# ivan-digital/qwen3-asr-swift

Hardware: AMD Instinct MI355X
Metric: audio-seconds/sec (RTF^-1) Qwen3-ASR-0.6B, 30 s@16 kHz, b=32 per GPU (higher is better)
Workload: dtype bf16; 1 GPU; Qwen3-ASR-0.6B geometry (bf16), 32 clips x 30 s per GPU (BASELINE metric's b=32; x8 GPUs = configs[2]), timed region = pcm in host memory -> mel + encoder + prompt pass + 128 forced greedy tokens -> token ids in host memory, tokens gathered over RCCL; clips_per_gpu=32, weights=bf16

## Files before the change

### qwen3-asr-swift_amd/csrc/dec_kernels.h

```cpp
#pragma once
#include "common.h"
#include "gemm.h"
#include "dec_rope.h"
#include <vector>

namespace qasr {

struct QuantRaw {
    const uint32_t* wq = nullptr;
    const void* scales = nullptr;
    const void* biases = nullptr;
    int sb_f32 = 0;
    int N = 0, K = 0, bits = 0;
};

void rmsnorm_rows_launch(const bf16_t* x, const bf16_t* w, bf16_t* y, int rows, int H, float eps, hipStream_t s);

void embed_splice_launch(const int* ids, const int* audio_src, const bf16_t* embed, const bf16_t* audio, bf16_t* x,
                         int n_pos, int H, hipStream_t s);

void gather_rows_launch(const bf16_t* src, const int* row_idx, bf16_t* dst, int n, int H, hipStream_t s);

struct KVLayout {
    bf16_t* k;
    bf16_t* v;
    int max_ctx, kv_heads, hd;
    bf16_t* vf = nullptr;
    __host__ __device__ long off(int slot, int kvh, int pos) const {
        return (((long)slot * kv_heads + kvh) * max_ctx + pos) * hd;
    }
};

void qk_norm_rope_launch(const bf16_t* qkv, const int* slot, const int* pos, int n_pos, int heads, int kv_heads,
                         int hd, const bf16_t* qn_w, const bf16_t* kn_w, float eps, const float* rope_cos,
                         const float* rope_sin, bf16_t* qr, KVLayout cache, bf16_t* vt, int vt_stride,
                         const int* cu, const int* slot_of_clip, int n_clips, int max_len, hipStream_t s, bool v_only = false);
bool qk_norm_rope_fusable(int heads, int kv_heads, int hd);

void prefill_attention_launch(const bf16_t* qr, KVLayout cache, const bf16_t* vt, int vt_stride, const int* cu,
                              const int* slot_of_clip, int n_clips, int max_len, int heads, bf16_t* out,
                              hipStream_t s, unsigned long long* dbg = nullptr);

enum DecEpi { DEC_EPI_BF16 = 0, DEC_EPI_RESID = 1, DEC_EPI_SWIGLU = 2, DEC_EPI_LOGITS = 3 };

struct DecGemvArgs {
    const bf16_t* W;
    const bf16_t* Wp;
    const bf16_t* X;
    int B, N, K;
    bf16_t* out;
    float* logits;
    float* part_val;
    int* part_idx;
};
int decode_gemv_launch(DecEpi epi, const DecGemvArgs& a, hipStream_t s);
int decode_gemv_blocks(DecEpi epi, int N);
void argmax_rows_launch(const bf16_t* x, long ld, int rows, int n, int* out, hipStream_t s);

void decode_gemv_set_debug(unsigned long long* dbg);
int decode_gemv_fused_launch(DecEpi epi, const DecGemvArgs& a, const bf16_t* norm_w, float eps, bf16_t* norm_scratch,
                             hipStream_t s);
void decode_gemv_note_route(int tuned);
int decode_gemv_last_route();

// ... 15 lines not shown
    int* ctx_len;
    int* n_active;
    int* err;
    int max_new;
    int max_tokens;
    int eos;
    int ignore_eos;
    int vocab;
    unsigned* clear = nullptr;
    int clear_words = 0;
};
struct RopeRows {
    const float* cos_table; const float* sin_table;
    float* cos_rows; float* sin_rows;
    int half;
};
void greedy_finalize_launch(const float* part_val, const int* part_idx, int n_parts, GreedyState st, int B,
                            int advance_ctx, const bf16_t* embed, bf16_t* x, int H, RopeRows rr, hipStream_t s,
                            const QuantRaw* qembed = nullptr);

void refresh_rope_rows_launch(const int* ctx_len, RopeRows rr, int B, hipStream_t s);
void rope_tables_host(float theta, int half, int n_pos, std::vector<float>& c, std::vector<float>& sn);

struct EpiQkHeads {
    bf16_t* qkv; long ldo;
    bf16_t* qr;
    KVLayout cache;
    const int* slot; const int* pos;
    const bf16_t* qn_w; const bf16_t* kn_w;
    float eps;
    const float* rope_cos; const float* rope_sin;
    int heads, kv_heads;
    __device__ __forceinline__ bool head_tile(int n0) const { return n0 < (heads + kv_heads) * 128; }
    __device__ __forceinline__ void operator()(int m, int n, float4 v) const {
        *reinterpret_cast<uint2*>(qkv + (long)m * ldo + n) = pack_bf16x4(v);
    }
    __device__ __forceinline__ void rows(int m0, int n0, int M, const unsigned short* T, int tid) const {
        constexpr int HD = 128, HALF = 64;
        const int h = n0 / HD, j = tid & 7;
        const bf16_t* nw = h < heads ? qn_w : kn_w;
        const uint4 w1 = *reinterpret_cast<const uint4*>(nw + 8 * j), w2 = *reinterpret_cast<const uint4*>(nw + HALF + 8 * j);
        const bf16_t* w1e = reinterpret_cast<const bf16_t*>(&w1);
        const bf16_t* w2e = reinterpret_cast<const bf16_t*>(&w2);
#pragma unroll
        for (int pass = 0; pass < 4; ++pass) {
            const int row = pass * 32 + (tid >> 3);
            const bool live = m0 + row < M;
            const int m = live ? m0 + row : M - 1;
            const int sw = (row >> 2) & 7;
            const uint4 a = *reinterpret_cast<const uint4*>(T + row * 128 + ((j ^ sw) << 3));
            const uint4 b = *reinterpret_cast<const uint4*>(T + row * 128 + (((8 + j) ^ sw) << 3));
            const bf16_t* ae = reinterpret_cast<const bf16_t*>(&a);
            const bf16_t* be = reinterpret_cast<const bf16_t*>(&b);
            const int sl = slot[m], ps = pos[m];
            float x1[8], x2[8], ss = 0.0f;
#pragma unroll
            for (int e = 0; e < 8; ++e) {
                x1[e] = bf16_to_f32(ae[e]);
                x2[e] = bf16_to_f32(be[e]);
                ss += x1[e] * x1[e] + x2[e] * x2[e];
            }
#pragma unroll
            for (int ofs = 1; ofs < 8; ofs <<= 1) ss += __shfl_xor(ss, ofs, 64);
            const float inv = rsqrtf(ss / (float)HD + eps);
            const float4* cp = reinterpret_cast<const float4*>(rope_cos + (long)ps * HALF + 8 * j);
            const float4* sp = reinterpret_cast<const float4*>(rope_sin + (long)ps * HALF + 8 * j);
            const float4 c0 = cp[0], c1 = cp[1], s0 = sp[0], s1 = sp[1];
            const float cs[8] = {c0.x, c0.y, c0.z, c0.w, c1.x, c1.y, c1.z, c1.w};
            const float sn[8] = {s0.x, s0.y, s0.z, s0.w, s1.x, s1.y, s1.z, s1.w};
            uint4 o1, o2;
            bf16_t* o1e = reinterpret_cast<bf16_t*>(&o1);
            bf16_t* o2e = reinterpret_cast<bf16_t*>(&o2);
#pragma unroll
            for (int e = 0; e < 8; ++e) {
                float r1, r2;
                norm_rope_pair(x1[e], x2[e], bf16_to_f32(w1e[e]), bf16_to_f32(w2e[e]), inv, cs[e], sn[e], r1, r2);
                o1e[e] = f32_to_bf16(r1);
                o2e[e] = f32_to_bf16(r2);
            }
            if (live) {
                bf16_t* dst = h < heads ? qr + ((long)m * heads + h) * HD : cache.k + cache.off(sl, h - heads, ps);
                *reinterpret_cast<uint4*>(dst + 8 * j) = o1;
                *reinterpret_cast<uint4*>(dst + HALF + 8 * j) = o2;
            }
        }
    }
};

struct EpiResidBf16 {
    bf16_t* x; long ldx;
    struct Pre { uint2 r; };
    __device__ __forceinline__ Pre prefetch(int m, int n) const { return {*reinterpret_cast<const uint2*>(x + (long)m * ldx + n)}; }
    __device__ __forceinline__ void apply(int m, int n, float4 v, const Pre& p) const {
        float4 r = unpack_bf16x4(p.r);
        r.x += bf16_round(v.x); r.y += bf16_round(v.y); r.z += bf16_round(v.z); r.w += bf16_round(v.w);
        *reinterpret_cast<uint2*>(x + (long)m * ldx + n) = pack_bf16x4(r);
    }
    __device__ __forceinline__ void operator()(int m, int n, float4 v) const { apply(m, n, v, prefetch(m, n)); }
};

__device__ __forceinline__ float swiglu_bf16(float g_acc, float u_acc) { return gemm_swiglu(g_acc, u_acc); }

}
```

### qwen3-asr-swift_amd/csrc/dec_prefill.hip

```cpp
#include "dec_kernels.h"
#include "dec_rope.h"
#include <cstdlib>
#include <cstdio>

namespace qasr {

constexpr int RMS_MAXV = 4;

__global__ __launch_bounds__(256) void rmsnorm_rows_kernel(const bf16_t* __restrict__ x, const bf16_t* __restrict__ w,
                                                           bf16_t* __restrict__ y, int rows, int H, float eps) {
    const int row = blockIdx.x * 4 + (threadIdx.x >> 6), lane = threadIdx.x & 63;
    if (row >= rows) return;
    const int nch = H / 8;
    const uint4* xr = reinterpret_cast<const uint4*>(x + (long)row * H);
    uint4 v[RMS_MAXV];
    float ss = 0.0f;
#pragma unroll
    for (int i = 0; i < RMS_MAXV; ++i) {
        int c = lane + 64 * i;
        v[i] = c < nch ? xr[c] : make_uint4(0, 0, 0, 0);
        const bf16_t* e = reinterpret_cast<const bf16_t*>(&v[i]);
#pragma unroll
        for (int j = 0; j < 8; ++j) { float f = bf16_to_f32(e[j]); ss = fmaf(f, f, ss); }
    }
// ... 221 lines not shown
        long waves = (long)n_pos * (nh / 2);
        hipLaunchKernelGGL(qk_norm_rope_kernel<128>, dim3(cdiv(waves, 4)), dim3(256), 0, s, qkv, slot, pos, n_pos, heads,
                           kv_heads, qn_w, kn_w, eps, rope_cos, rope_sin, qr, cache);
        hipLaunchKernelGGL(v_transpose_kernel<128>, tgrid, dim3(256), 0, s, cache, qkv, nh, heads + kv_heads, cu, slot_of_clip, vt_out, vt_stride);
    } else if (hd == 32 && nh % 8 == 0) {
        long waves = (long)n_pos * (nh / 8);
        hipLaunchKernelGGL(qk_norm_rope_kernel<32>, dim3(cdiv(waves, 4)), dim3(256), 0, s, qkv, slot, pos, n_pos, heads,
                           kv_heads, qn_w, kn_w, eps, rope_cos, rope_sin, qr, cache);
        hipLaunchKernelGGL(v_transpose_kernel<32>, tgrid, dim3(256), 0, s, cache, qkv, nh, heads + kv_heads, cu, slot_of_clip, vt_out, vt_stride);
    } else {
        throw std::invalid_argument("qk_norm_rope: unsupported (head_dim, head count)");
    }
}

bool qk_norm_rope_fusable(int heads, int kv_heads, int hd) {
    return hd == 128 && (heads + kv_heads) % 8 == 0 && tuning().qknr_wide != 0 && tuning().pp_fuse_qk != 0;
}

template <int HD, int MT>
__global__ __launch_bounds__(256) void prefill_attention_kernel(const bf16_t* __restrict__ qr, KVLayout cache,
                                                                const bf16_t* __restrict__ vt, int vt_stride,
                                                                const int* __restrict__ cu,
                                                                const int* __restrict__ slot_of_clip, int heads,
                                                                bf16_t* __restrict__ out, float scale) {
    constexpr int KT = 64;
    constexpr int KCH = HD / 8;
    constexpr int KS = HD / 32;
    constexpr int DT = HD / 16;
    constexpr int PLD = KT + 8;
    constexpr int NKL = KT * KCH / 256;
    constexpr int NVL = HD * (KT / 8) / 256;
    static_assert(KT * KCH % 256 == 0 && HD * (KT / 8) % 256 == 0, "tile staging must divide evenly");
    __shared__ __attribute__((aligned(16))) bf16_t s_kv[2 * KT * HD];
    __shared__ __attribute__((aligned(16))) bf16_t s_p[4][16 * MT][PLD];
    bf16_t* s_k = s_kv;
    bf16_t* s_v = s_kv + KT * HD;
    constexpr int QW = 16 * MT, QB = 4 * QW;
    const int clip = blockIdx.z, h = blockIdx.y, q0 = blockIdx.x * QB;
    const int row0 = cu[clip], T = cu[clip + 1] - row0;
    if (q0 >= T) return;
    const int tid = threadIdx.x, lane = tid & 63, wave = tid >> 6, fr = lane & 15, fc = lane >> 4;
    const int sl = slot_of_clip[clip];
    const int kvh = h / (heads / cache.kv_heads);
    const bf16_t* kbase = cache.k + cache.off(sl, kvh, 0);
    const bf16_t* vbase = vt + ((long)sl * cache.kv_heads + kvh) * HD * vt_stride;
    const int qw = q0 + wave * QW;

    auto stage = [&](int k0) {
        uint4 kreg[NKL], vreg[NVL];
#pragma unroll
        for (int i = 0; i < NKL; ++i) {
            const int idx = tid + i * 256, key = idx / KCH, ch = idx - key * KCH;
            const int kc = k0 + key < T ? k0 + key : T - 1;
            kreg[i] = *reinterpret_cast<const uint4*>(kbase + (long)kc * HD + ch * 8);
            if (k0 + key >= T) kreg[i] = make_uint4(0, 0, 0, 0);
        }
#pragma unroll
        for (int i = 0; i < NVL; ++i) {
            const int idx = tid + i * 256, d = idx / (KT / 8), ch = idx - d * (KT / 8);
            vreg[i] = *reinterpret_cast<const uint4*>(vbase + (long)d * vt_stride + k0 + ch * 8);
        }
#pragma unroll
// ... 116 lines not shown
    for (int mi = 0; mi < MT; ++mi)
#pragma unroll
        for (int j = 0; j < 4; ++j) {
            const float invl = 1.0f / l_run[mi][j];
            const int r = mi * 16 + fc * 4 + j;
#pragma unroll
            for (int d = 0; d < DT; ++d) s_o[r * HD + d * 16 + fr] = f32_to_bf16(o[mi][d][j] * invl);
        }
    __builtin_amdgcn_fence(__ATOMIC_RELEASE, "wavefront");
    __builtin_amdgcn_wave_barrier();
    for (int i = lane; i < QW * KCH; i += 64) {
        const int r = i / KCH, ch = i - r * KCH;
        if (qw + r < T)
            *reinterpret_cast<uint4*>(out + ((long)(row0 + qw + r) * heads + h) * HD + ch * 8) =
                *reinterpret_cast<const uint4*>(&s_o[r * HD + ch * 8]);
    }
}

template <int HD, bool VFRAG, bool STAMPS = false>
__global__ __launch_bounds__(256) __attribute__((amdgpu_waves_per_eu(2, 2))) void prefill_attention2_kernel(const bf16_t* __restrict__ qr, KVLayout cache,
                                                                 const bf16_t* __restrict__ vt, int vt_stride,
                                                                 const int* __restrict__ cu,
                                                                 const int* __restrict__ slot_of_clip, int heads,
                                                                 bf16_t* __restrict__ out, float scale, int heavy_first,
                                                                 unsigned long long* __restrict__ dbg = nullptr) {
    [[maybe_unused]] unsigned long long st_t0 = 0, st_prev = 0, st_sum[6] = {0, 0, 0, 0, 0, 0};
#define PA_MARK(p) do { if constexpr (STAMPS) { const unsigned long long t_ = wall_clock64(); st_sum[p] += t_ - st_prev; st_prev = t_; } } while (0)
    if constexpr (STAMPS) { st_t0 = wall_clock64(); st_prev = st_t0; }
    constexpr int KT = 64, KS = HD / 32, DT = HD / 16, KCH = HD / 8, REP = 2;
    constexpr int TILE_BYTES = KT * HD * 2;
    constexpr int K_RPI = 64 / KCH, K_IPW = KT / K_RPI / 4;
    constexpr int V_IPW = HD / 8 / 4;
    static_assert(K_IPW >= 1 && V_IPW >= 1, "tile staging geometry");
    typedef __attribute__((address_space(3))) void* lds_ptr_t;
    typedef const __attribute__((address_space(1))) void* glb_ptr_t;
    __shared__ __attribute__((aligned(16))) char smem[2][2][TILE_BYTES];
    const int clip = heavy_first ? blockIdx.y : blockIdx.z, kvh = heavy_first ? blockIdx.x : blockIdx.y;
    const int q0 = (heavy_first ? gridDim.z - 1 - blockIdx.z : blockIdx.x) * 64;
    const int row0 = cu[clip], T = cu[clip + 1] - row0;
    if (q0 >= T) return;
    const int tid = threadIdx.x, lane = tid & 63, wave = tid >> 6, fr = lane & 15, g = lane >> 4;
    const int sl = slot_of_clip[clip];
    const bf16_t* kbase = cache.k + cache.off(sl, kvh, 0);
    const bf16_t* vbase = vt + ((long)sl * cache.kv_heads + kvh) * HD * vt_stride;
    const int qw = q0 + wave * 16, qpos = qw + fr;

    unsigned koff[K_IPW], voff[V_IPW];
#pragma unroll
    for (int i = 0; i < K_IPW; ++i) {
        const int r = (wave * K_IPW + i) * K_RPI + lane / KCH, c = lane % KCH;
        koff[i] = (unsigned)(r * HD + ((c ^ (r & (KCH - 1))) << 3)) * 2u;
    }
#pragma unroll
    for (int i = 0; i < V_IPW; ++i) {
        const int inst = wave * V_IPW + i;
        if (VFRAG) voff[i] = (unsigned)(inst * 1024 + lane * 16);
        else {
            const int d = inst * 8 + (lane >> 3), c = lane & 7;
            voff[i] = (unsigned)(d * vt_stride + ((c ^ (d & 7)) << 3)) * 2u;
        }
    }
    const char* vsrc = VFRAG ? reinterpret_cast<const char*>(cache.vf + cache.off(sl, kvh, 0)) : reinterpret_cast<const char*>(vbase);
// ... 163 lines not shown
            for (int i = 0; i < 6; ++i) d[2 + i] = st_sum[i];
        }
    }
#undef PA_MARK
    if (qpos < T) {
#pragma unroll
        for (int mi = 0; mi < REP; ++mi) {
            float l = l_run[mi];
            l += __shfl_xor(l, 16, 64);
            l += __shfl_xor(l, 32, 64);
            const float invl = 1.0f / l;
            bf16_t* dst = out + ((long)(row0 + qpos) * heads + kvh * REP + mi) * HD + g * 4;
#pragma unroll
            for (int d = 0; d < DT; ++d) {
                const uint2 v = make_uint2(pack_bf16x2(o[mi][d][0] * invl, o[mi][d][1] * invl), pack_bf16x2(o[mi][d][2] * invl, o[mi][d][3] * invl));
                *reinterpret_cast<uint2*>(dst + d * 16) = v;
            }
        }
    }
}

void prefill_attention_launch(const bf16_t* qr, KVLayout cache, const bf16_t* vt, int vt_stride, const int* cu,
                              const int* slot_of_clip, int n_clips, int max_len, int heads, bf16_t* out,
                              hipStream_t s, unsigned long long* dbg) {
    if (n_clips <= 0 || max_len <= 0) return;
    const int mt = tuning().pa_mt;
    const int form = tuning().pa_form;
    const float scale = 1.0f / sqrtf((float)cache.hd);
    if (form >= 2 && heads == 2 * cache.kv_heads && (cache.hd == 128 || cache.hd == 32)) {
        const int hf = tuning().pa_order != 0 && cache.kv_heads == 8 ? 1 : 0;
        const dim3 grid = hf ? dim3(cache.kv_heads, n_clips, cdiv(max_len, 64)) : dim3(cdiv(max_len, 64), cache.kv_heads, n_clips);
        const bool vfrag = cache.vf != nullptr && tuning().pa_vfrag != 0;
        if (dbg) {
            if (cache.hd != 128 || !vfrag) throw std::invalid_argument("prompt attention stamps: head_dim 128 with the fragment image only");
            hipLaunchKernelGGL((prefill_attention2_kernel<128, true, true>), grid, dim3(256), 0, s, qr, cache, vt, vt_stride, cu, slot_of_clip, heads, out, scale, hf, dbg);
            return;
        }
        if (cache.hd == 128) {
            if (vfrag) hipLaunchKernelGGL((prefill_attention2_kernel<128, true>), grid, dim3(256), 0, s, qr, cache, vt, vt_stride, cu, slot_of_clip, heads, out, scale, hf);
            else hipLaunchKernelGGL((prefill_attention2_kernel<128, false>), grid, dim3(256), 0, s, qr, cache, vt, vt_stride, cu, slot_of_clip, heads, out, scale, hf);
        } else {
            if (vfrag) hipLaunchKernelGGL((prefill_attention2_kernel<32, true>), grid, dim3(256), 0, s, qr, cache, vt, vt_stride, cu, slot_of_clip, heads, out, scale, hf);
            else hipLaunchKernelGGL((prefill_attention2_kernel<32, false>), grid, dim3(256), 0, s, qr, cache, vt, vt_stride, cu, slot_of_clip, heads, out, scale, hf);
        }
        return;
    }
    if (cache.hd == 128 && mt == 2)
        hipLaunchKernelGGL((prefill_attention_kernel<128, 2>), dim3(cdiv(max_len, 128), heads, n_clips), dim3(256), 0, s,
                           qr, cache, vt, vt_stride, cu, slot_of_clip, heads, out, scale);
    else if (cache.hd == 128)
        hipLaunchKernelGGL((prefill_attention_kernel<128, 1>), dim3(cdiv(max_len, 64), heads, n_clips), dim3(256), 0, s,
                           qr, cache, vt, vt_stride, cu, slot_of_clip, heads, out, scale);
    else if (cache.hd == 32)
        hipLaunchKernelGGL((prefill_attention_kernel<32, 2>), dim3(cdiv(max_len, 128), heads, n_clips), dim3(256), 0, s,
                           qr, cache, vt, vt_stride, cu, slot_of_clip, heads, out, scale);
    else
        throw std::invalid_argument("prefill attention: head_dim must be 32 or 128");
}

}
```

### qwen3-asr-swift_amd/csrc/decoder.hip

```cpp
#include "engine.h"
#include "dec_sampler.h"
#include "dec_chain.h"
#include "dec_gemv_wide.h"
#include <algorithm>
#include <cmath>
#include <cstring>
#include <cstdlib>
#include <cstdio>

namespace qasr {

__global__ void interleave_gate_up_kernel(const bf16_t* __restrict__ gate, const bf16_t* __restrict__ up,
                                          bf16_t* __restrict__ dst, int inter, int H) {
    const int r = blockIdx.x;
    const int blk = r >> 5, w = r & 31;
    const bf16_t* src = (w < 16 ? gate : up) + (long)(blk * 16 + (w & 15)) * H;
    const uint4* s4 = reinterpret_cast<const uint4*>(src);
    uint4* d4 = reinterpret_cast<uint4*>(dst + (long)r * H);
    for (int i = threadIdx.x; i < H / 8; i += blockDim.x) d4[i] = s4[i];
}

__global__ void interleave_rows_bytes_kernel(const char* __restrict__ a, const char* __restrict__ b, char* __restrict__ dst,
                                             int row_bytes) {
    const int r = blockIdx.x, blk = r >> 5, w = r & 31;
// ... 217 lines not shown
    QASR_HIP(hipMemsetAsync(d_vt_.p, 0, d_vt_.bytes, stream_));
    d_px_.alloc((size_t)max_pos_ * H * 2);
    d_ph_.alloc((size_t)max_pos_ * H * 2);
    d_pqkv_.alloc((size_t)max_pos_ * nh * hd * 2);
    d_pqr_.alloc((size_t)max_pos_ * nq * 2);
    d_pattn_.alloc((size_t)max_pos_ * nq * 2);
    d_pact_.alloc((size_t)max_pos_ * I * 2);
    d_dx_.alloc((size_t)B * H * 2);
    d_dh_.alloc((size_t)B * H * 2);
    d_dqkv_.alloc((size_t)B * nh * hd * 2);
    d_dattn_.alloc((size_t)B * nq * 2);
    d_dact_.alloc((size_t)B * I * 2);
    d_chain_ctr_.alloc(CHAIN_STATE_BYTES);
    QASR_HIP(hipMemsetAsync(d_chain_ctr_.p, 0, CHAIN_STATE_BYTES, stream_));
    d_qa_gran_.alloc(QA_GRAN_BYTES);
    QASR_HIP(hipMemsetAsync(d_qa_gran_.p, 0, QA_GRAN_BYTES, stream_));
    d_qa_part_.alloc(QA_PART_BYTES);
    QASR_HIP(hipMemsetAsync(d_qa_part_.p, 0, QA_PART_BYTES, stream_));
    d_logits_.alloc((size_t)B * cfg_.vocab * sizeof(float));
    n_parts_ = decw_.quant ? lm_head_q_parts(cfg_.vocab, H, cfg_.bits) : lm_head_parts(cfg_.vocab, H);
    const int parts_cap = std::max(n_parts_, decode_gemv_blocks(DEC_EPI_LOGITS, cfg_.vocab));
    d_part_val_.alloc((size_t)B * parts_cap * sizeof(float));
    d_part_idx_.alloc((size_t)B * parts_cap * sizeof(int));
    const size_t pmeta = (size_t)max_pos_ * 4 * sizeof(int) + (size_t)(3 * B + 2) * sizeof(int);
    h_pmeta_.alloc(pmeta);
    d_pmeta_.alloc(pmeta);
    const size_t gs = ((size_t)B * (cfg_.max_new_tokens + 1) + 3 * B + 4) * sizeof(int);
    d_gstate_.alloc(gs);
    int* g = d_gstate_.as<int>();
    gstate_.tokens = g;
    gstate_.lens = g + (size_t)B * (cfg_.max_new_tokens + 1);
    gstate_.finished = gstate_.lens + B;
    gstate_.ctx_len = gstate_.finished + B;
    gstate_.n_active = gstate_.ctx_len + B;
    gstate_.err = gstate_.n_active + 1;
    d_err_flag_ = gstate_.err;
    gstate_.max_new = cfg_.max_new_tokens;
    gstate_.eos = cfg_.tok_im_end;
    gstate_.vocab = cfg_.vocab;
    gstate_.clear = d_chain_ctr_.as<unsigned>();
    gstate_.clear_words = (int)(CHAIN_CTR_BYTES / sizeof(unsigned));
    for (auto& e : ev_)
        if (!e) QASR_HIP(hipEventCreate(&e));
    QASR_HIP(hipStreamSynchronize(stream_));
}

void Engine::plan_prefill(const qasr_options* opt, const std::vector<int>& n_audio,
// ... 5 lines not shown
    if (n_ctx + n_lang > cfg_.max_prompt_extra) throw std::length_error("context + language ids exceed max_prompt_extra");
    auto check_ids = [&](const int32_t* ids, int n, const char* what) {
        for (int i = 0; i < n; ++i)
            if (ids[i] < 0 || ids[i] >= cfg_.vocab)
                throw std::invalid_argument(std::string(what) + " id " + std::to_string(ids[i]) + " outside [0, vocab)");
    };
    if (n_ctx) check_ids(opt->context_ids, n_ctx, "context");
    if (n_lang) check_ids(opt->language_ids, n_lang, "language");
    if (aligner_tails)
        for (auto& t : *aligner_tails) check_ids(t.data(), (int)t.size(), "slotted text");
    if (aligner_tails) {
        if ((int)aligner_tails->size() != B) throw std::invalid_argument("aligner: one slotted text per clip");
        for (auto& t : *aligner_tails)
            if ((int)t.size() > cfg_.max_prompt_extra) throw std::length_error("slotted text exceeds max_prompt_extra");
    }
    char* hp = h_pmeta_.as<char>();
    int* ids = reinterpret_cast<int*>(hp);
    int* asrc = ids + max_pos_;
    int* slot = asrc + max_pos_;
    int* pos = slot + max_pos_;
    int* cu = pos + max_pos_;
    int* slotclip = cu + (B + 1);
    int* last = slotclip + B;
    int p = 0;
    max_len_ = 0;
    prompt_len_.assign(B, 0);
    cu[0] = 0;
    for (int b = 0; b < B; ++b) {
        const int start = p;
        auto push = [&](int id, int a) { ids[p] = id; asrc[p] = a; slot[p] = b; pos[p] = p - start; ++p; };
        push(cfg_.tok_im_start, -1); push(cfg_.tok_system, -1); push(cfg_.tok_newline, -1);
        for (int i = 0; i < n_ctx; ++i) push(opt->context_ids[i], -1);
        push(cfg_.tok_im_end, -1); push(cfg_.tok_newline, -1);
        push(cfg_.tok_im_start, -1); push(cfg_.tok_user, -1); push(cfg_.tok_newline, -1); push(cfg_.tok_audio_start, -1);
        for (int i = 0; i < n_audio[b]; ++i) push(cfg_.tok_audio_pad, clip_tok_off_[b] + i);
        push(cfg_.tok_audio_end, -1); push(cfg_.tok_im_end, -1); push(cfg_.tok_newline, -1);
        push(cfg_.tok_im_start, -1); push(cfg_.tok_assistant, -1); push(cfg_.tok_newline, -1);
        if (aligner_tails) {
            for (int32_t id : (*aligner_tails)[b]) push(id, -1);
        } else {
            for (int i = 0; i < n_lang; ++i) push(opt->language_ids[i], -1);
            push(cfg_.tok_asr_text, -1);
        }
        prompt_len_[b] = p - start;
        if (prompt_len_[b] > max_prompt_) throw std::length_error("prompt longer than engine capacity");
        max_len_ = std::max(max_len_, prompt_len_[b]);
        cu[b + 1] = p;
        slotclip[b] = b;
        last[b] = p - 1;
    }
    n_pos_ = p;
    const size_t bytes = (size_t)max_pos_ * 4 * sizeof(int) + (size_t)(3 * B + 1) * sizeof(int);
    QASR_HIP(hipMemcpyAsync(d_pmeta_.p, h_pmeta_.p, bytes, hipMemcpyHostToDevice, stream_));
    int* dp = d_pmeta_.as<int>();
    d_p_ids_ = dp;
    d_p_audio_src_ = dp + max_pos_;
    d_p_slot_ = dp + 2 * (size_t)max_pos_;
    d_p_pos_ = dp + 3 * (size_t)max_pos_;
    d_p_cu_ = dp + 4 * (size_t)max_pos_;
    d_p_slotclip_ = d_p_cu_ + (B + 1);
    d_p_last_ = d_p_slotclip_ + B;
    h_ctx0_ = prompt_len_;
}

void Engine::reset_greedy_state(int max_tokens, bool ignore_eos) {
    const int B = batch_;
    cur_max_tokens_ = max_tokens;
    cur_ignore_eos_ = ignore_eos;
    gstate_.max_tokens = max_tokens;
    gstate_.ignore_eos = ignore_eos ? 1 : 0;
    QASR_HIP(hipMemsetAsync(gstate_.tokens, 0xff, (size_t)cfg_.max_batch * (cfg_.max_new_tokens + 1) * sizeof(int), stream_));
    QASR_HIP(hipMemsetAsync(gstate_.lens, 0, (size_t)2 * cfg_.max_batch * sizeof(int), stream_));
    if (!h_ginit_.p) h_ginit_.alloc((size_t)(cfg_.max_batch + 2) * sizeof(int));
    int* init = h_ginit_.as<int>();
    for (int b = 0; b < cfg_.max_batch; ++b) init[b] = b < B ? h_ctx0_[b] : 0;
    init[cfg_.max_batch] = B;
    init[cfg_.max_batch + 1] = 0;
    QASR_HIP(hipMemcpyAsync(gstate_.ctx_len, init, (size_t)(cfg_.max_batch + 2) * sizeof(int), hipMemcpyHostToDevice, stream_));
    steps_done_ = 0;
    forced_steps_ = 0;
    forced_ready_ = false;
}

void Engine::run_lm_head(bool want_logits, int r0, int nr, hipStream_t s) {
// ... 24 lines not shown
    bf16_t* wqkv = d_wscratch_.as<bf16_t>();
    bf16_t* wo = wqkv + (size_t)(nq + 2 * nkv) * H;
    bf16_t* wgu = wo + (size_t)H * nq;
    bf16_t* wdown = wgu + (size_t)2 * I * H;
    const DequantJob jobs[7] = {{L.rq, 0, nq, wqkv},
                                {L.rk, 0, nkv, wqkv + (size_t)nq * H},
                                {L.rv, 0, nkv, wqkv + (size_t)(nq + nkv) * H},
                                {L.ro, 0, H, wo},
                                {L.rg, 0, I, wgu, 16, 32, 0},
                                {L.ru, 0, I, wgu, 16, 32, 16},
                                {L.rd, 0, H, wdown}};
    quant_dequant_multi_launch(jobs, 7, s);
    return {wqkv, wo, wgu, wdown};
}

void Engine::run_prefill(bool want_logits) {
    const int H = cfg_.hidden, hd = cfg_.head_dim, nq = cfg_.heads * hd, nh = cfg_.heads + 2 * cfg_.kv_heads, I = cfg_.inter;
    hipStream_t s = stream_;
    bf16_t *x = d_px_.as<bf16_t>(), *h = d_ph_.as<bf16_t>(), *qkv = d_pqkv_.as<bf16_t>(), *qr = d_pqr_.as<bf16_t>();
    bf16_t *at = d_pattn_.as<bf16_t>(), *act = d_pact_.as<bf16_t>();
    const int P = n_pos_;
    if (decw_.quant) embed_splice_q_launch(d_p_ids_, d_p_audio_src_, decw_.embed_raw, d_audio_.as<bf16_t>(), x, P, H, s);
    else embed_splice_launch(d_p_ids_, d_p_audio_src_, decw_.embed, d_audio_.as<bf16_t>(), x, P, H, s);
    for (int l = 0; l < cfg_.dec_layers; ++l) {
        const DecLayerW& L = decw_.layers[l];
        const bool aligner = cfg_.classify_num > 0;
        KVLayout kv{kcache_[aligner ? 0 : l]->as<bf16_t>(), nullptr, max_ctx_, cfg_.kv_heads, hd,
                    aligner ? nullptr : vfcache_[l]->as<bf16_t>()};
        const PromptW W = prompt_weights(l, s);
        rmsnorm_rows_launch(x, L.ln1, h, P, H, cfg_.rms_eps, s);
        const bool fuse_qk = qk_norm_rope_fusable(cfg_.heads, cfg_.kv_heads, hd);
        if (fuse_qk)
            gemm_nt_headtiles(ADense{h, H, P, H}, W.wqkv, H, P, nh * hd, H,
                              EpiQkHeads{qkv, (long)nh * hd, qr, kv, d_p_slot_, d_p_pos_, L.qn, L.kn, cfg_.rms_eps, d_rope_cos_.as<float>(),
                                         d_rope_sin_.as<float>(), cfg_.heads, cfg_.kv_heads}, s);
        else
            gemm_nt(ADense{h, H, P, H}, W.wqkv, H, P, nh * hd, H, EpiStoreBf16{qkv, (long)nh * hd}, s);
        qk_norm_rope_launch(qkv, d_p_slot_, d_p_pos_, P, cfg_.heads, cfg_.kv_heads, hd, L.qn, L.kn, cfg_.rms_eps,
                            d_rope_cos_.as<float>(), d_rope_sin_.as<float>(), qr, kv, d_vt_.as<bf16_t>(), vt_stride_,
                            d_p_cu_, d_p_slotclip_, batch_, max_len_, s, fuse_qk);
        prefill_attention_launch(qr, kv, d_vt_.as<bf16_t>(), vt_stride_, d_p_cu_, d_p_slotclip_, batch_, max_len_,
                                 cfg_.heads, at, s);
        gemm_nt(ADense{at, nq, P, nq}, W.wo, nq, P, H, nq, EpiResidBf16{x, H}, s);
        rmsnorm_rows_launch(x, L.ln2, h, P, H, cfg_.rms_eps, s);
        gemm_nt_swiglu(ADense{h, H, P, H}, W.wgu, H, P, 2 * I, H, EpiStoreBf16{act, I}, s);
        gemm_nt(ADense{act, I, P, I}, W.wdown, I, P, H, I, EpiResidBf16{x, H}, s);
    }
    if (cfg_.classify_num > 0) { QASR_HIP(hipGetLastError()); return; }
    gather_rows_launch(x, d_p_last_, d_dx_.as<bf16_t>(), batch_, H, s);
    run_lm_head(want_logits, 0, batch_, s);
    QASR_HIP(hipGetLastError());
}

void Engine::align_forward(const float* const* pcm, const size_t* n, size_t B,
// ... 822 lines not shown
```

### qwen3-asr-swift_amd/csrc/engine.h

```cpp
#pragma once
#include "common.h"
#include "mel.h"
#include "enc_kernels.h"
#include "dec_kernels.h"
#include "dec_quant.h"
#include "qasr.h"
#include <map>
#include <memory>
#include <string>
#include <unordered_map>
#include <vector>

namespace qasr {

struct DevBuf {
    void* p = nullptr;
    size_t bytes = 0;
    DevBuf() = default;
    DevBuf(const DevBuf&) = delete;
    DevBuf& operator=(const DevBuf&) = delete;
    ~DevBuf() { release(); }
    void alloc(size_t n) {
        release();
        if (n == 0) n = 16;
// ... 220 lines not shown
        QuantRaw embed_raw{};
        QuantImg embed_q{};
        std::vector<DecLayerW> layers;
    } decw_;
    int max_prompt_ = 0, max_ctx_ = 0, max_pos_ = 0, vt_stride_ = 0;
    DevBuf d_rope_cos_, d_rope_sin_, d_rope_rows_;
    std::vector<std::unique_ptr<DevBuf>> kcache_, vfcache_;
    unsigned long long* stamp_buf_ = nullptr;
    int stamp_layer_ = -1;
    DevBuf d_al_rows_, d_al_x_, d_al_logits_, d_al_idx_;
    DevBuf d_vt_;
    DevBuf d_px_, d_ph_, d_pqkv_, d_pqr_, d_pattn_, d_pact_;
    DevBuf d_dx_, d_dh_, d_dqkv_, d_dattn_, d_dact_, d_logits_, d_part_val_, d_part_idx_;
    bool shared_device_ = false;
    unsigned long long* qa_dbg_ = nullptr;
    unsigned long long* chain_dbg_ = nullptr;
    DevBuf d_qa_part_;
    DevBuf d_qa_gran_;
    DevBuf d_chain_ctr_;
    HostBuf h_pmeta_;
    DevBuf d_pmeta_;
    int *d_p_ids_ = nullptr, *d_p_audio_src_ = nullptr, *d_p_slot_ = nullptr, *d_p_pos_ = nullptr;
    int *d_p_cu_ = nullptr, *d_p_slotclip_ = nullptr, *d_p_last_ = nullptr;
    int n_pos_ = 0, max_len_ = 0;
    std::vector<int> prompt_len_;
    DevBuf d_gstate_;
    GreedyState gstate_{};
    int cur_max_tokens_ = 448;
    bool cur_ignore_eos_ = false;
    int n_parts_ = 0;
    int steps_done_ = 0;
    hipGraphExec_t graph_exec_ = nullptr;
    hipGraphExec_t graph_exec_n_ = nullptr;
    int graph_n_ = 0;
    long graph_key_ = -1;
    unsigned graph_epoch_ = 0;
    int* d_err_flag_ = nullptr;
    int forced_steps_ = 0;
    bool forced_ready_ = false;
    void forced_step(const int* d_ids, int B);
    void drop_graph();
    void require_batch(const char* what) const;
    hipEvent_t ev_[6] = {};
    hipStream_t side_[3] = {};
    hipEvent_t fork_ev_ = nullptr, join_ev_[3] = {};
    std::vector<int> h_ctx0_;
    HostBuf h_ginit_;
// ... 24 lines not shown
```

### qwen3-asr-swift_amd/csrc/tuning.cpp

```cpp
#include "tuning.h"
#include <cctype>
#include <cstdio>
#include <cstdlib>
#include <cstring>
#include <string>

namespace qasr {

namespace {
struct Entry { const char* key; int Tuning::*field; int allowed[6]; bool diag_only; };
const Entry kEntries[] = {
    {"gemv_splitb", &Tuning::gemv_splitb, {0, 1, 2, -1}, false}, {"gemv_xbar", &Tuning::gemv_xbar, {0, 1, 2, 3, 4, -1}, false}, {"gemv_w1024", &Tuning::gemv_w1024, {4, 8, -1}, false},
    {"gemv_nt", &Tuning::gemv_nt, {0, 1, -1}, false}, {"lmh_nt", &Tuning::lmh_nt, {0, 1, -1}, false},
    {"gemv_wide", &Tuning::gemv_wide, {0, 1, -1}, false}, {"gemv_earlyw", &Tuning::gemv_earlyw, {0, 1, 2, 3, -1}, false}, {"gemv_partial", &Tuning::gemv_partial, {0, 1, -1}, false},
    {"chain", &Tuning::chain, {0, 1, 2, 3, -1}, false}, {"chain_fault", &Tuning::chain_fault, {0, 1, -1}, false}, {"chain_proto", &Tuning::chain_proto, {0, 1, -1}, false}, {"chain_pf", &Tuning::chain_pf, {0, 1, -1}, false}, {"qa", &Tuning::qa, {0, 1, -1}, false},
    {"qa_early", &Tuning::qa_early, {0, 5, -2}, false}, {"qa_gate", &Tuning::qa_gate, {0, 1, 2, -1}, false}, {"qa_gran", &Tuning::qa_gran, {0, 1, -1}, false}, {"qa_split", &Tuning::qa_split, {0, 1, 2, -1}, false}, {"qa_xbar", &Tuning::qa_xbar, {0, 1, 2, -1}, false},
    {"da_unr", &Tuning::da_unr, {1, 2, -1}, false},
    {"da_waves", &Tuning::da_waves, {8, 16, -1}, false}, {"da_spec", &Tuning::da_spec, {0, 1, 2, 3, -1}, false}, {"da_earlyq", &Tuning::da_earlyq, {0, 1, -1}, false},
    {"pa_form", &Tuning::pa_form, {1, 2, -1}, false}, {"pa_mt", &Tuning::pa_mt, {1, 2, -1}, false}, {"pa_order", &Tuning::pa_order, {0, 1, -1}, false}, {"pa_vfrag", &Tuning::pa_vfrag, {0, 1, -1}, false},
    {"pp_fuse_qk", &Tuning::pp_fuse_qk, {0, 1, -1}, false}, {"qknr_wide", &Tuning::qknr_wide, {0, 1, -1}, false},
    {"tts_packed_prompt", &Tuning::tts_packed_prompt, {0, 1, -1}, false}, {"codec_tail_rows", &Tuning::codec_tail_rows, {0, 1, -1}, false}, {"cvlm_prompt_chunk", &Tuning::cvlm_prompt_chunk, {1, 64, -1}, false},
    {"vae_fuse_c", &Tuning::vae_fuse_c, {0, 128, -2}, false}, {"vloc_skinny_rows", &Tuning::vloc_skinny_rows, {0, 256, -2}, false},
    {"conv_ktile", &Tuning::conv_ktile, {0, 1, -1}, false}, {"enc_attn", &Tuning::enc_attn, {0, 1, -1}, false}, {"mha_form", &Tuning::mha_form, {0, 1, 2, -1}, false},
    {"gemm_p8", &Tuning::gemm_p8, {0, 1, 2, -1}, false}, {"gemm_nbuf", &Tuning::gemm_nbuf, {0, 1, 2, -1}, false}, {"gemm_tm", &Tuning::gemm_tm, {1, 4, 8, 16, -1}, false},
    {"lmh_q_ring", &Tuning::lmh_q_ring, {0, 1, -1}, false}, {"lmh_grid", &Tuning::lmh_grid, {1, 4096, -2}, false}, {"lmh_order", &Tuning::lmh_order, {0, 1, -1}, false},
    {"lmh_diag", &Tuning::lmh_diag, {0, 1, -1}, true},
    {"decode_split", &Tuning::decode_split, {1, 4, -2}, false}, {"decode_gran", &Tuning::decode_gran, {16, 32, 48, 64, -1}, false},
    {"graph_steps", &Tuning::graph_steps, {1, 2, 4, 8, -1}, false}, {"use_graph", &Tuning::use_graph, {0, 1, -1}, false},
    {"device_sampler", &Tuning::device_sampler, {0, 1, -1}, false},
    {"da_stamps", &Tuning::da_stamps, {0, 1, -1}, true}, {"gemv_stamps", &Tuning::gemv_stamps, {0, 1, -1}, true},
    {"stamps_insitu", &Tuning::stamps_insitu, {0, 1, -1}, true}, {"pa_stamps", &Tuning::pa_stamps, {0, 1, -1}, true},
};

bool value_allowed(const Entry& e, int v) {
#ifndef QASR_DIAG_STAMPS
    if (e.diag_only && v != 0) return false;
#endif
    if (e.allowed[2] == -2) return v >= e.allowed[0] && v <= e.allowed[1];
    for (int i = 0; i < 6 && e.allowed[i] != -1; ++i)
        if (e.allowed[i] == v) return true;
    return false;
}
}
// ... 41 lines not shown
```

### qwen3-asr-swift_amd/csrc/tuning.h

```cpp
#pragma once

namespace qasr {

struct Tuning {
    int gemv_xbar = 4;
    int gemv_splitb = 2;
    int gemv_w1024 = 8;
    int gemv_partial = 1;
    int gemv_earlyw = 1;
    int gemv_nt = 0;
    int lmh_nt = 1;
    int gemv_wide = 1;
    int chain = 0;
    int qa = 1;
    int qa_early = 5;
    int qa_xbar = 2;
    int qa_split = 1;
    int qa_gran = 1;
    int qa_gate = 2;
    int chain_fault = 0;
    int chain_proto = 0;
    int chain_pf = 0;
    int da_unr = 2;
    int da_waves = 8;
    int da_spec = 3;
    int da_earlyq = 0;
    int pa_form = 2;
    int pa_vfrag = 1;
    int pa_order = 1;
    int pa_mt = 1;
    int pp_fuse_qk = 1;
    int qknr_wide = 1;
    int tts_packed_prompt = 1;
    int cvlm_prompt_chunk = 64;
    int codec_tail_rows = 1;
    int vae_fuse_c = 64;
    int vloc_skinny_rows = 256;
    int conv_ktile = 1;
    int enc_attn = 1;
    int mha_form = 1;
    int gemm_p8 = 1;
    int gemm_tm = 8;
    int gemm_nbuf = 0;
    int lmh_q_ring = 1;
    int lmh_order = 1;
    int lmh_grid = 256;
    int lmh_diag = 0;
    int decode_split = 1;
    int decode_gran = 16;
    int graph_steps = 8;
    int use_graph = 1;
    int device_sampler = 1;
    int da_stamps = 0, gemv_stamps = 0, stamps_insitu = 0, pa_stamps = 0;
    unsigned epoch = 0;
// ... 10 lines not shown
```

Before: 6379 audio-seconds/sec.

## Compute only last-token rows in final prompt decoder layer

In the last decoder layer of the prompt pass, K/V is still projected for every position, but Q is projected only for rows in each clip's final query tile. Attention runs only on that last tile per clip, and the output projection, MLP and LM head run only on the final token of each clip. The goal is to skip most of the last layer's Q projection, attention and MLP work, which does not affect the next-token logits. It adds row-map metadata, an extra gather and a templated epilogue, and it depends on the query-tile size matching the attention kernel's tiling.

Result: no change. 6403 audio-seconds/sec (median of 6 runs) (+0.4%).

```diff
diff --git a/qwen3-asr-swift_amd/csrc/dec_kernels.h b/qwen3-asr-swift_amd/csrc/dec_kernels.h
--- a/qwen3-asr-swift_amd/csrc/dec_kernels.h
+++ b/qwen3-asr-swift_amd/csrc/dec_kernels.h
@@ -39,7 +39,8 @@
 
 void prefill_attention_launch(const bf16_t* qr, KVLayout cache, const bf16_t* vt, int vt_stride, const int* cu,
                               const int* slot_of_clip, int n_clips, int max_len, int heads, bf16_t* out,
-                              hipStream_t s, unsigned long long* dbg = nullptr);
+                              hipStream_t s, unsigned long long* dbg = nullptr, bool last_tile = false);
+int prefill_attention_qtile(int heads, int kv_heads, int hd);
 
 enum DecEpi { DEC_EPI_BF16 = 0, DEC_EPI_RESID = 1, DEC_EPI_SWIGLU = 2, DEC_EPI_LOGITS = 3 };
 
@@ -101,7 +102,8 @@
 void refresh_rope_rows_launch(const int* ctx_len, RopeRows rr, int B, hipStream_t s);
 void rope_tables_host(float theta, int half, int n_pos, std::vector<float>& c, std::vector<float>& sn);
 
-struct EpiQkHeads {
+template <bool MAP>
+struct EpiQkHeadsT {
     bf16_t* qkv; long ldo;
     bf16_t* qr;
     KVLayout cache;
@@ -110,6 +112,7 @@
     float eps;
     const float* rope_cos; const float* rope_sin;
     int heads, kv_heads;
+    const int* rowmap = nullptr;
     __device__ __forceinline__ bool head_tile(int n0) const { return n0 < (heads + kv_heads) * 128; }
     __device__ __forceinline__ void operator()(int m, int n, float4 v) const {
         *reinterpret_cast<uint2*>(qkv + (long)m * ldo + n) = pack_bf16x4(v);
@@ -125,7 +128,8 @@
         for (int pass = 0; pass < 4; ++pass) {
             const int row = pass * 32 + (tid >> 3);
             const bool live = m0 + row < M;
-            const int m = live ? m0 + row : M - 1;
+            const int mg = live ? m0 + row : M - 1;
+            const int m = MAP ? rowmap[mg] : mg;
             const int sw = (row >> 2) & 7;
             const uint4 a = *reinterpret_cast<const uint4*>(T + row * 128 + ((j ^ sw) << 3));
             const uint4 b = *reinterpret_cast<const uint4*>(T + row * 128 + (((8 + j) ^ sw) << 3));
@@ -165,6 +169,7 @@
         }
     }
 };
+using EpiQkHeads = EpiQkHeadsT<false>;
 
 struct EpiResidBf16 {
     bf16_t* x; long ldx;
diff --git a/qwen3-asr-swift_amd/csrc/dec_prefill.hip b/qwen3-asr-swift_amd/csrc/dec_prefill.hip
--- a/qwen3-asr-swift_amd/csrc/dec_prefill.hip
+++ b/qwen3-asr-swift_amd/csrc/dec_prefill.hip
@@ -267,7 +267,7 @@
                                                                 const bf16_t* __restrict__ vt, int vt_stride,
                                                                 const int* __restrict__ cu,
                                                                 const int* __restrict__ slot_of_clip, int heads,
-                                                                bf16_t* __restrict__ out, float scale) {
+                                                                bf16_t* __restrict__ out, float scale, int last_tile) {
     constexpr int KT = 64;
     constexpr int KCH = HD / 8;
     constexpr int KS = HD / 32;
@@ -281,8 +281,9 @@
     bf16_t* s_k = s_kv;
     bf16_t* s_v = s_kv + KT * HD;
     constexpr int QW = 16 * MT, QB = 4 * QW;
-    const int clip = blockIdx.z, h = blockIdx.y, q0 = blockIdx.x * QB;
+    const int clip = blockIdx.z, h = blockIdx.y;
     const int row0 = cu[clip], T = cu[clip + 1] - row0;
+    const int q0 = (last_tile ? (T - 1) / QB : (int)blockIdx.x) * QB;
     if (q0 >= T) return;
     const int tid = threadIdx.x, lane = tid & 63, wave = tid >> 6, fr = lane & 15, fc = lane >> 4;
     const int sl = slot_of_clip[clip];
@@ -445,7 +446,7 @@
                                                                  const bf16_t* __restrict__ vt, int vt_stride,
                                                                  const int* __restrict__ cu,
                                                                  const int* __restrict__ slot_of_clip, int heads,
-                                                                 bf16_t* __restrict__ out, float scale, int heavy_first,
+                                                                 bf16_t* __restrict__ out, float scale, int heavy_first, int last_tile,
                                                                  unsigned long long* __restrict__ dbg = nullptr) {
     [[maybe_unused]] unsigned long long st_t0 = 0, st_prev = 0, st_sum[6] = {0, 0, 0, 0, 0, 0};
 #define PA_MARK(p) do { if constexpr (STAMPS) { const unsigned long long t_ = wall_clock64(); st_sum[p] += t_ - st_prev; st_prev = t_; } } while (0)
@@ -459,8 +460,8 @@
     typedef const __attribute__((address_space(1))) void* glb_ptr_t;
     __shared__ __attribute__((aligned(16))) char smem[2][2][TILE_BYTES];
     const int clip = heavy_first ? blockIdx.y : blockIdx.z, kvh = heavy_first ? blockIdx.x : blockIdx.y;
-    const int q0 = (heavy_first ? gridDim.z - 1 - blockIdx.z : blockIdx.x) * 64;
     const int row0 = cu[clip], T = cu[clip + 1] - row0;
+    const int q0 = (last_tile ? (T - 1) / 64 : heavy_first ? (int)(gridDim.z - 1 - blockIdx.z) : (int)blockIdx.x) * 64;
     if (q0 >= T) return;
     const int tid = threadIdx.x, lane = tid & 63, wave = tid >> 6, fr = lane & 15, g = lane >> 4;
     const int sl = slot_of_clip[clip];
@@ -670,8 +671,10 @@
 
 void prefill_attention_launch(const bf16_t* qr, KVLayout cache, const bf16_t* vt, int vt_stride, const int* cu,
                               const int* slot_of_clip, int n_clips, int max_len, int heads, bf16_t* out,
-                              hipStream_t s, unsigned long long* dbg) {
+                              hipStream_t s, unsigned long long* dbg, bool last_tile) {
     if (n_clips <= 0 || max_len <= 0) return;
+    const int lt = last_tile ? 1 : 0;
+    if (last_tile) max_len = 1;
     const int mt = tuning().pa_mt;
     const int form = tuning().pa_form;
     const float scale = 1.0f / sqrtf((float)cache.hd);
@@ -681,29 +684,35 @@
         const bool vfrag = cache.vf != nullptr && tuning().pa_vfrag != 0;
         if (dbg) {
             if (cache.hd != 128 || !vfrag) throw std::invalid_argument("prompt attention stamps: head_dim 128 with the fragment image only");
-            hipLaunchKernelGGL((prefill_attention2_kernel<128, true, true>), grid, dim3(256), 0, s, qr, cache, vt, vt_stride, cu, slot_of_clip, heads, out, scale, hf, dbg);
+            hipLaunchKernelGGL((prefill_attention2_kernel<128, true, true>), grid, dim3(256), 0, s, qr, cache, vt, vt_stride, cu, slot_of_clip, heads, out, scale, hf, lt, dbg);
             return;
         }
         if (cache.hd == 128) {
-            if (vfrag) hipLaunchKernelGGL((prefill_attention2_kernel<128, true>), grid, dim3(256), 0, s, qr, cache, vt, vt_stride, cu, slot_of_clip, heads, out, scale, hf);
-            else hipLaunchKernelGGL((prefill_attention2_kernel<128, false>), grid, dim3(256), 0, s, qr, cache, vt, vt_stride, cu, slot_of_clip, heads, out, scale, hf);
+            if (vfrag) hipLaunchKernelGGL((prefill_attention2_kernel<128, true>), grid, dim3(256), 0, s, qr, cache, vt, vt_stride, cu, slot_of_clip, heads, out, scale, hf, lt);
+            else hipLaunchKernelGGL((prefill_attention2_kernel<128, false>), grid, dim3(256), 0, s, qr, cache, vt, vt_stride, cu, slot_of_clip, heads, out, scale, hf, lt);
         } else {
-            if (vfrag) hipLaunchKernelGGL((prefill_attention2_kernel<32, true>), grid, dim3(256), 0, s, qr, cache, vt, vt_stride, cu, slot_of_clip, heads, out, scale, hf);
-            else hipLaunchKernelGGL((prefill_attention2_kernel<32, false>), grid, dim3(256), 0, s, qr, cache, vt, vt_stride, cu, slot_of_clip, heads, out, scale, hf);
+            if (vfrag) hipLaunchKernelGGL((prefill_attention2_kernel<32, true>), grid, dim3(256), 0, s, qr, cache, vt, vt_stride, cu, slot_of_clip, heads, out, scale, hf, lt);
+            else hipLaunchKernelGGL((prefill_attention2_kernel<32, false>), grid, dim3(256), 0, s, qr, cache, vt, vt_stride, cu, slot_of_clip, heads, out, scale, hf, lt);
         }
         return;
     }
     if (cache.hd == 128 && mt == 2)
         hipLaunchKernelGGL((prefill_attention_kernel<128, 2>), dim3(cdiv(max_len, 128), heads, n_clips), dim3(256), 0, s,
-                           qr, cache, vt, vt_stride, cu, slot_of_clip, heads, out, scale);
+                           qr, cache, vt, vt_stride, cu, slot_of_clip, heads, out, scale, lt);
     else if (cache.hd == 128)
         hipLaunchKernelGGL((prefill_attention_kernel<128, 1>), dim3(cdiv(max_len, 64), heads, n_clips), dim3(256), 0, s,
-                           qr, cache, vt, vt_stride, cu, slot_of_clip, heads, out, scale);
+                           qr, cache, vt, vt_stride, cu, slot_of_clip, heads, out, scale, lt);
     else if (cache.hd == 32)
         hipLaunchKernelGGL((prefill_attention_kernel<32, 2>), dim3(cdiv(max_len, 128), heads, n_clips), dim3(256), 0, s,
-                           qr, cache, vt, vt_stride, cu, slot_of_clip, heads, out, scale);
+                           qr, cache, vt, vt_stride, cu, slot_of_clip, heads, out, scale, lt);
     else
         throw std::invalid_argument("prefill attention: head_dim must be 32 or 128");
 }
 
-}
+int prefill_attention_qtile(int heads, int kv_heads, int hd) {
+    if (tuning().pa_form >= 2 && heads == 2 * kv_heads && (hd == 128 || hd == 32)) return 64;
+    if (hd == 128) return tuning().pa_mt == 2 ? 128 : 64;
+    return 128;
+}
+
+}
diff --git a/qwen3-asr-swift_amd/csrc/decoder.hip b/qwen3-asr-swift_amd/csrc/decoder.hip
--- a/qwen3-asr-swift_amd/csrc/decoder.hip
+++ b/qwen3-asr-swift_amd/csrc/decoder.hip
@@ -263,7 +263,7 @@
     const int parts_cap = std::max(n_parts_, decode_gemv_blocks(DEC_EPI_LOGITS, cfg_.vocab));
     d_part_val_.alloc((size_t)B * parts_cap * sizeof(float));
     d_part_idx_.alloc((size_t)B * parts_cap * sizeof(int));
-    const size_t pmeta = (size_t)max_pos_ * 4 * sizeof(int) + (size_t)(3 * B + 2) * sizeof(int);
+    const size_t pmeta = (size_t)max_pos_ * 4 * sizeof(int) + (size_t)(3 * B + 2) * sizeof(int) + (size_t)128 * B * sizeof(int);
     h_pmeta_.alloc(pmeta);
     d_pmeta_.alloc(pmeta);
     const size_t gs = ((size_t)B * (cfg_.max_new_tokens + 1) + 3 * B + 4) * sizeof(int);
@@ -315,6 +315,9 @@
     int* cu = pos + max_pos_;
     int* slotclip = cu + (B + 1);
     int* last = slotclip + B;
+    int* qrows = last + B;
+    p_qtile_ = prefill_attention_qtile(cfg_.heads, cfg_.kv_heads, cfg_.head_dim);
+    n_qrows_ = 0;
     int p = 0;
     max_len_ = 0;
     prompt_len_.assign(B, 0);
@@ -341,9 +344,10 @@
         cu[b + 1] = p;
         slotclip[b] = b;
         last[b] = p - 1;
+        for (int r = start + (prompt_len_[b] - 1) / p_qtile_ * p_qtile_; r < p; ++r) qrows[n_qrows_++] = r;
     }
     n_pos_ = p;
-    const size_t bytes = (size_t)max_pos_ * 4 * sizeof(int) + (size_t)(3 * B + 1) * sizeof(int);
+    const size_t bytes = (size_t)max_pos_ * 4 * sizeof(int) + (size_t)(3 * B + 1 + n_qrows_) * sizeof(int);
     QASR_HIP(hipMemcpyAsync(d_pmeta_.p, h_pmeta_.p, bytes, hipMemcpyHostToDevice, stream_));
     int* dp = d_pmeta_.as<int>();
     d_p_ids_ = dp;
@@ -353,6 +357,7 @@
     d_p_cu_ = dp + 4 * (size_t)max_pos_;
     d_p_slotclip_ = d_p_cu_ + (B + 1);
     d_p_last_ = d_p_slotclip_ + B;
+    d_p_qrows_ = d_p_last_ + B;
     h_ctx0_ = prompt_len_;
 }
 
@@ -423,6 +428,8 @@
     const int P = n_pos_;
     if (decw_.quant) embed_splice_q_launch(d_p_ids_, d_p_audio_src_, decw_.embed_raw, d_audio_.as<bf16_t>(), x, P, H, s);
     else embed_splice_launch(d_p_ids_, d_p_audio_src_, decw_.embed, d_audio_.as<bf16_t>(), x, P, H, s);
+    const bool last_rows = tuning().pp_last_rows != 0 && cfg_.classify_num == 0 &&
+                           p_qtile_ == prefill_attention_qtile(cfg_.heads, cfg_.kv_heads, hd);
     for (int l = 0; l < cfg_.dec_layers; ++l) {
         const DecLayerW& L = decw_.layers[l];
         const bool aligner = cfg_.classify_num > 0;
@@ -431,6 +438,34 @@
         const PromptW W = prompt_weights(l, s);
         rmsnorm_rows_launch(x, L.ln1, h, P, H, cfg_.rms_eps, s);
         const bool fuse_qk = qk_norm_rope_fusable(cfg_.heads, cfg_.kv_heads, hd);
+        if (last_rows && l == cfg_.dec_layers - 1) {
+            const int B = batch_, nkv = cfg_.kv_heads * hd;
+            bf16_t *hq = act, *at_l = qkv, *h_l = h, *act_l = act, *x_l = d_dx_.as<bf16_t>();
+            if (fuse_qk) {
+                gemm_nt_headtiles(ADense{h, H, P, H}, W.wqkv + (size_t)nq * H, H, P, 2 * nkv, H,
+                                  EpiQkHeads{qkv + nq, (long)nh * hd, qr, kv, d_p_slot_, d_p_pos_, L.qn, L.kn, cfg_.rms_eps, d_rope_cos_.as<float>(),
+                                             d_rope_sin_.as<float>(), 0, cfg_.kv_heads}, s);
+                gather_rows_launch(h, d_p_qrows_, hq, n_qrows_, H, s);
+                gemm_nt_headtiles(ADense{hq, H, n_qrows_, H}, W.wqkv, H, n_qrows_, nq, H,
+                                  EpiQkHeadsT<true>{nullptr, 0, qr, kv, d_p_slot_, d_p_pos_, L.qn, L.kn, cfg_.rms_eps, d_rope_cos_.as<float>(),
+                                                    d_rope_sin_.as<float>(), cfg_.heads, 0, d_p_qrows_}, s);
+            } else {
+                gemm_nt(ADense{h, H, P, H}, W.wqkv, H, P, nh * hd, H, EpiStoreBf16{qkv, (long)nh * hd}, s);
+            }
+            qk_norm_rope_launch(qkv, d_p_slot_, d_p_pos_, P, cfg_.heads, cfg_.kv_heads, hd, L.qn, L.kn, cfg_.rms_eps,
+                                d_rope_cos_.as<float>(), d_rope_sin_.as<float>(), qr, kv, d_vt_.as<bf16_t>(), vt_stride_,
+                                d_p_cu_, d_p_slotclip_, B, max_len_, s, fuse_qk);
+            prefill_attention_launch(qr, kv, d_vt_.as<bf16_t>(), vt_stride_, d_p_cu_, d_p_slotclip_, B, max_len_, cfg_.heads, at, s, nullptr, true);
+            gather_rows_launch(x, d_p_last_, x_l, B, H, s);
+            gather_rows_launch(at, d_p_last_, at_l, B, nq, s);
+            gemm_nt(ADense{at_l, nq, B, nq}, W.wo, nq, B, H, nq, EpiResidBf16{x_l, H}, s);
+            rmsnorm_rows_launch(x_l, L.ln2, h_l, B, H, cfg_.rms_eps, s);
+            gemm_nt_swiglu(ADense{h_l, H, B, H}, W.wgu, H, B, 2 * I, H, EpiStoreBf16{act_l, I}, s);
+            gemm_nt(ADense{act_l, I, B, I}, W.wdown, I, B, H, I, EpiResidBf16{x_l, H}, s);
+            run_lm_head(want_logits, 0, B, s);
+            QASR_HIP(hipGetLastError());
+            return;
+        }
         if (fuse_qk)
             gemm_nt_headtiles(ADense{h, H, P, H}, W.wqkv, H, P, nh * hd, H,
                               EpiQkHeads{qkv, (long)nh * hd, qr, kv, d_p_slot_, d_p_pos_, L.qn, L.kn, cfg_.rms_eps, d_rope_cos_.as<float>(),
diff --git a/qwen3-asr-swift_amd/csrc/engine.h b/qwen3-asr-swift_amd/csrc/engine.h
--- a/qwen3-asr-swift_amd/csrc/engine.h
+++ b/qwen3-asr-swift_amd/csrc/engine.h
@@ -266,7 +266,8 @@
     DevBuf d_pmeta_;
     int *d_p_ids_ = nullptr, *d_p_audio_src_ = nullptr, *d_p_slot_ = nullptr, *d_p_pos_ = nullptr;
     int *d_p_cu_ = nullptr, *d_p_slotclip_ = nullptr, *d_p_last_ = nullptr;
-    int n_pos_ = 0, max_len_ = 0;
+    int* d_p_qrows_ = nullptr;
+    int n_pos_ = 0, max_len_ = 0, n_qrows_ = 0, p_qtile_ = 64;
     std::vector<int> prompt_len_;
     DevBuf d_gstate_;
     GreedyState gstate_{};
diff --git a/qwen3-asr-swift_amd/csrc/tuning.cpp b/qwen3-asr-swift_amd/csrc/tuning.cpp
--- a/qwen3-asr-swift_amd/csrc/tuning.cpp
+++ b/qwen3-asr-swift_amd/csrc/tuning.cpp
@@ -18,7 +18,7 @@
     {"da_unr", &Tuning::da_unr, {1, 2, -1}, false},
     {"da_waves", &Tuning::da_waves, {8, 16, -1}, false}, {"da_spec", &Tuning::da_spec, {0, 1, 2, 3, -1}, false}, {"da_earlyq", &Tuning::da_earlyq, {0, 1, -1}, false},
     {"pa_form", &Tuning::pa_form, {1, 2, -1}, false}, {"pa_mt", &Tuning::pa_mt, {1, 2, -1}, false}, {"pa_order", &Tuning::pa_order, {0, 1, -1}, false}, {"pa_vfrag", &Tuning::pa_vfrag, {0, 1, -1}, false},
-    {"pp_fuse_qk", &Tuning::pp_fuse_qk, {0, 1, -1}, false}, {"qknr_wide", &Tuning::qknr_wide, {0, 1, -1}, false},
+    {"pp_fuse_qk", &Tuning::pp_fuse_qk, {0, 1, -1}, false}, {"pp_last_rows", &Tuning::pp_last_rows, {0, 1, -1}, false},{"qknr_wide", &Tuning::qknr_wide, {0, 1, -1}, false},
     {"tts_packed_prompt", &Tuning::tts_packed_prompt, {0, 1, -1}, false}, {"codec_tail_rows", &Tuning::codec_tail_rows, {0, 1, -1}, false}, {"cvlm_prompt_chunk", &Tuning::cvlm_prompt_chunk, {1, 64, -1}, false},
     {"vae_fuse_c", &Tuning::vae_fuse_c, {0, 128, -2}, false}, {"vloc_skinny_rows", &Tuning::vloc_skinny_rows, {0, 256, -2}, false},
     {"conv_ktile", &Tuning::conv_ktile, {0, 1, -1}, false}, {"enc_attn", &Tuning::enc_attn, {0, 1, -1}, false}, {"mha_form", &Tuning::mha_form, {0, 1, 2, -1}, false},
diff --git a/qwen3-asr-swift_amd/csrc/tuning.h b/qwen3-asr-swift_amd/csrc/tuning.h
--- a/qwen3-asr-swift_amd/csrc/tuning.h
+++ b/qwen3-asr-swift_amd/csrc/tuning.h
@@ -30,6 +30,7 @@
     int pa_order = 1;
     int pa_mt = 1;
     int pp_fuse_qk = 1;
+    int pp_last_rows = 1;
     int qknr_wide = 1;
     int tts_packed_prompt = 1;
     int cvlm_prompt_chunk = 64;
```
